# aikiriao/LINNE

Hardware: AMD Instinct MI355X
Metric: frames/sec encode (-m 7) + decode, 44.1 kHz stereo, bit-exact; 1/2/4/8 GPU (higher is better)
Workload: dtype f64; 1 GPU; encode -m 7: 1 x 60 min 44.1 kHz int16 2-channel per GPU = 15504 frames of 10240 samples (tail 9280), MS on, PCM resident in HBM; decode = inverse hot path on the encode output; frames_per_gpu=15504, channels=2, preset=7, tracks_per_gpu=1

## Files before the change

### linne_amd/csrc/lnn_k_finalize.h

```cpp
#ifndef LNN_K_FINALIZE_H_INCLUDED
#define LNN_K_FINALIZE_H_INCLUDED

#define FIN_THREADS 256
#define FIN_TILE (4 * FIN_THREADS)
#define FIN_HALO (LNN_MAXL * LNN_MAXP)

__global__ __launch_bounds__(64) void k_quantize(Plan p)
{
    __shared__ uint32_t s_best;
    const uint32_t cf = blockIdx.x, tid = threadIdx.x;
    const size_t ocf = (size_t)p.frame_map[cf / p.C] * p.C + cf % p.C;
    int32_t *rec = p.prm + ocf * LINNE_AMD_PARAM_WORDS;
    double *st = p.stats + ocf * LINNE_AMD_STAT_WORDS;
    if (tid == 0) {
        double min_loss = (double)FLT_MAX; uint32_t best = 0;
        for (uint32_t r = 0; r < p.R; r++) { const double l = p.jloss[(size_t)cf * p.R + r]; if (l < min_loss) { min_loss = l; best = r; } }
        s_best = best;
        st[LINNE_AMD_ST_TAIL] = p.jtail[(size_t)cf * p.R + best];
        st[LINNE_AMD_ST_BEST] = p.af_best ? (double)p.af_best[cf] : (double)best;
        st[LINNE_AMD_ST_LOSS] = p.af_loss ? p.af_loss[cf] : p.jloss[(size_t)cf * p.R + best];
    }
    uint32_t used = LINNE_AMD_PRM_COEF;
    for (uint32_t l = 0; l < p.L; l++) used += p.P[l];
    for (uint32_t i = LINNE_AMD_PRM_UNITS + tid; i < LINNE_AMD_PARAM_WORDS; i += 64u)
        if ((i >= LINNE_AMD_PRM_UNITS + p.L && i < LINNE_AMD_PRM_RSHIFT) || (i >= LINNE_AMD_PRM_RSHIFT + p.L && i < LINNE_AMD_PRM_COEF) || i >= used) rec[i] = 0;
    __syncthreads();
    const uint32_t job = cf * p.R + s_best;
    __shared__ double s_d[LNN_MAXL][LNN_MAXP];
    for (uint32_t i = tid; i < p.L * LNN_MAXP; i += 64u) { const uint32_t l = i / LNN_MAXP, k = i % LNN_MAXP; if (k < p.P[l]) s_d[l][k] = p.lparams[((size_t)job * LNN_MAXL + l) * LNN_MAXP + k]; }
    __syncthreads();
    if (tid < p.L) {
        const uint32_t l = tid, P = p.P[l];
        const double *d = s_d[l];
        int32_t *cq = rec + LINNE_AMD_PRM_COEF + p.coef_off[l];
        double mx = 0.0;
        for (uint32_t k = 0; k < P; k++) if (mx < fabs(d[k])) mx = fabs(d[k]);
        uint32_t rshift;
        if (mx <= 0.0078125) {
            rshift = 8;
            for (uint32_t k = 0; k < P; k++) cq[k] = 0;
        } else {
            int ndigit; (void)frexp(mx, &ndigit);
            rshift = (uint32_t)(7 - ndigit);
            const double sc = ldexp(1.0, (int)rshift);
            double qerr = 0.0;
            for (int32_t k = (int32_t)P - 1; k >= 0; k--) {
                qerr += d[k] * sc;
                int32_t q = (int32_t)round_away(qerr);
                if (q >= 128) q = 127; else if (q < -128) q = -128;
                qerr -= (double)q;
                cq[k] = q;
            }
        }
        rec[LINNE_AMD_PRM_UNITS + l] = (int32_t)p.lunits[(size_t)job * LNN_MAXL + l];
        rec[LINNE_AMD_PRM_RSHIFT + l] = (int32_t)rshift;
    }
}

#define FIN_FRONT 192u
#define FIN_BUF (FIN_FRONT + ((FIN_HALO + 63u) & ~63u) + FIN_TILE)
__global__ __launch_bounds__(FIN_THREADS, 4) void k_fir_cascade(Plan p)
{
    __shared__ __attribute__((aligned(16))) int32_t s_coef[LNN_MAXL][LNN_MAXP];
    __shared__ __attribute__((aligned(16))) int32_t bufs[2][FIN_BUF];
    __shared__ __attribute__((aligned(16))) int8_t dig[2][4][FIN_BUF];
    const uint32_t cf = blockIdx.x, tid = threadIdx.x;
    const uint32_t lane = tid & 63u, wave = (uint32_t)__builtin_amdgcn_readfirstlane((int)(tid >> 6));
    const DevClass &c = p.cls[p.cls_of_frame[cf / p.C]];
    const uint32_t n = c.n, S = p.S, L = p.L;
    const size_t ocf = (size_t)p.frame_map[cf / p.C] * p.C + cf % p.C;
    const int32_t *rec = p.prm + ocf * LINNE_AMD_PARAM_WORDS;
    int32_t *out = p.resid + ocf * S;
    uint32_t H = 0;
    for (uint32_t l = 0; l < L; l++) H += p.P[l];
    __shared__ uint32_t l_units[LNN_MAXL], l_rs[LNN_MAXL], l_matrix[LNN_MAXL + 1], s_toep_unit[LNN_MAXL];
    __shared__ lnn_v4i s_toep[LNN_MAXL][3][64];
    if (tid <= LNN_MAXL) {
        const uint32_t l = tid;
        if (l < LNN_MAXL) s_toep_unit[l] = 0xFFFFFFFFu;
        uint32_t m = 0;
        if (l < L) {
            const uint32_t units = (uint32_t)rec[LINNE_AMD_PRM_UNITS + l];
            l_units[l] = units; l_rs[l] = (uint32_t)rec[LINNE_AMD_PRM_RSHIFT + l];
            if (l > 0 && units != 0 && p.P[l] <= 128u) { const uint32_t np = p.P[l] / units; m = (np >= 16u && n / units >= np) ? 1u : 0u; }
        }
        l_matrix[l] = m;
    }
    const uint32_t ORG = FIN_FRONT + ((H + 63u) & ~63u);
    const int32_t *src = p.xint + (size_t)cf * S;
    const uint32_t ntile = (S + FIN_TILE - 1u) / FIN_TILE;
    constexpr int NPF = (FIN_HALO + FIN_TILE + FIN_THREADS - 1) / FIN_THREADS;
    int32_t pf[NPF];
    auto fetch = [&](uint32_t s0_) {
#pragma unroll
        for (int m = 0; m < NPF; m++) {
            const uint32_t i = tid + (uint32_t)m * FIN_THREADS;
            const int64_t g = (int64_t)s0_ - H + i;
            pf[m] = (i < H + FIN_TILE && g >= 0 && g < (int64_t)n) ? src[g] : 0;
        }
    };
    if (blockIdx.y < ntile && blockIdx.y * FIN_TILE < n) fetch(blockIdx.y * FIN_TILE);
    for (uint32_t i = tid; i < L * LNN_MAXP; i += FIN_THREADS) { const uint32_t l = i / LNN_MAXP, k = i % LNN_MAXP; if (k < p.P[l]) s_coef[l][k] = rec[LINNE_AMD_PRM_COEF + p.coef_off[l] + k]; }
    for (uint32_t tile = blockIdx.y; tile < ntile; tile += gridDim.y) {
    const uint32_t s0 = tile * FIN_TILE;
    if (s0 >= n) {
        for (uint32_t i = tid; i < FIN_TILE; i += FIN_THREADS) if (s0 + i < S) out[s0 + i] = 0;
        continue;
    }
    __syncthreads();
#pragma unroll
    for (int m = 0; m < NPF; m++) { const uint32_t i = tid + (uint32_t)m * FIN_THREADS; if (i < H + FIN_TILE) bufs[0][ORG - H + i] = pf[m]; }
    { const uint32_t tn = tile + gridDim.y; if (tn < ntile && tn * FIN_TILE < n) fetch(tn * FIN_TILE); }
    __syncthreads();
    uint32_t lead = H;
#pragma unroll 1
    for (uint32_t l = 0; l < L; l++) {
        const uint32_t units = l_units[l], rs = l_rs[l];
        const uint32_t np = p.P[l] / (units ? units : 1u), ns = units ? n / units : 0u;
        const uint32_t half = 1u << ((rs - 1u) & 31u);
        const bool last = (l + 1 == L), digits_out = l_matrix[l + 1] != 0;
        const int32_t *in = bufs[l & 1u];
        int32_t *ob = bufs[(l & 1u) ^ 1u];
        int8_t (*dgo)[FIN_BUF] = dig[(l & 1u) ^ 1u];
        const uint32_t olead = lead - p.P[l];
        const uint32_t count = olead + FIN_TILE;
        const uint32_t nsd = ns ? ns : 1u;
        auto scalar_out = [&](uint32_t idx) -> int32_t {
            const int64_t s64 = (int64_t)s0 - ORG + idx;
            if (s64 < 0 || s64 >= (int64_t)n) return 0;
            const uint32_t s = (uint32_t)s64, unit = s / nsd;
            int32_t v = in[idx];
            if (units && ns >= np && unit < units) {
                const uint32_t loc = s - unit * ns;
                if (loc >= np) {
                    uint32_t pred = half;
                    const int32_t *cc = s_coef[l] + unit * np;
                    const int32_t *xx = in + idx - np;
                    for (uint32_t k = 0; k < np; k++) pred += (uint32_t)cc[k] * (uint32_t)xx[k];
                    v = (int32_t)((uint32_t)v + (uint32_t)((int32_t)pred >> (rs & 31u)));
                }
            }
            return v;
        };
        auto put_digits = [&](uint32_t idx, int32_t v) {
            const uint32_t dg = sp_digits(v);
            dgo[0][idx] = (int8_t)dg; dgo[1][idx] = (int8_t)(dg >> 8); dgo[2][idx] = (int8_t)(dg >> 16); dgo[3][idx] = (int8_t)(dg >> 24);
        };
        if (l_matrix[l] != 0) {
            const uint32_t KS = (np + 15u + 63u) / 64u;
            const int8_t (*dgi)[FIN_BUF] = dig[l & 1u];
            const uint32_t first = (ORG - olead) & ~63u, nchunk = (ORG + FIN_TILE - first) / 64u;
            const uint32_t i = lane & 15u, g4 = lane >> 4, qa = (lane & 15u) >> 2, ba = lane & 3u;
            auto build_band = [&](uint32_t unit, lnn_v4i *frag) {
                const int32_t *cc = s_coef[l] + unit * np;
#pragma unroll
                for (uint32_t st = 0; st < 3u; st++) {
                    uint32_t w[4] = { 0u, 0u, 0u, 0u };
                    if (st < KS) {
#pragma unroll
                        for (uint32_t e = 0; e < 16u; e++) {
                            const int32_t kx = (int32_t)(64u * st + 16u * g4 + e + 16u + np) - (int32_t)(64u * KS + i);
                            const int32_t cv = (kx >= 0 && (uint32_t)kx < np) ? cc[kx] : 0;
                            w[e >> 2] |= ((uint32_t)cv & 0xFFu) << (8u * (e & 3u));
                        }
                    }
                    frag[st][0] = (int)w[0]; frag[st][1] = (int)w[1]; frag[st][2] = (int)w[2]; frag[st][3] = (int)w[3];
                }
            };
            const uint32_t u0 = ((s0 > olead) ? (s0 - olead) / nsd : 0u) < units ? ((s0 > olead) ? (s0 - olead) / nsd : 0u) : units - 1u;
            {
                const uint32_t held = s_toep_unit[l];
                __syncthreads();
                if (held != u0) {
                    if (wave == 0) { lnn_v4i fr[3]; build_band(u0, fr); s_toep[l][0][lane] = fr[0]; s_toep[l][1][lane] = fr[1]; s_toep[l][2][lane] = fr[2]; }
                    if (tid == 0) s_toep_unit[l] = u0;
                }
                __syncthreads();
            }
            lnn_v4i bfrag[3];
            uint32_t have_unit = 0xFFFFFFFFu;
            for (uint32_t ck = wave; ck < nchunk; ck += FIN_THREADS / 64u) {
                const uint32_t bc = first + 64u * ck;
                const int64_t sa = (int64_t)s0 - ORG + bc, sz = sa + 63;
                const uint32_t idx = bc + 16u * g4 + i;
                int32_t o;
                bool mat = sa >= 0 && sz < (int64_t)n;
                uint32_t unit = 0;
                if (mat) { unit = (uint32_t)sa / nsd; mat = unit < units && (uint32_t)sz / nsd == unit; }
                if (mat) {
                    if (unit != have_unit) {
                        if (unit == u0) { bfrag[0] = s_toep[l][0][lane]; bfrag[1] = s_toep[l][1][lane]; bfrag[2] = s_toep[l][2][lane]; }
                        else build_band(unit, bfrag);
                        have_unit = unit;
                    }
                    lnn_v4i acc4 = { 0, 0, 0, 0 };
                    const uint32_t w0 = bc + 16u * qa + 16u - 64u * KS + 16u * g4;
#pragma unroll
                    for (uint32_t st = 0; st < 3u; st++) {
                        if (st < KS) {
                            const lnn_v4i a = *(const lnn_v4i *)&dgi[ba][w0 + 64u * st];
                            acc4 = __builtin_amdgcn_mfma_i32_16x16x64_i8(a, bfrag[st], acc4, 0, 0, 0);
                        }
                    }
                    const uint32_t sum = (uint32_t)acc4[0] + ((uint32_t)acc4[1] << 8) + ((uint32_t)acc4[2] << 16) + ((uint32_t)acc4[3] << 24);
                    const uint32_t s = (uint32_t)((int64_t)s0 - ORG + idx), loc = s - unit * ns;
                    const int32_t v = in[idx];
                    o = (loc >= np) ? (int32_t)((uint32_t)v + (uint32_t)((int32_t)(half + sum) >> (rs & 31u))) : v;
                } else o = scalar_out(idx);
                if (last) { const int64_t s64 = (int64_t)s0 - ORG + idx; if (s64 >= (int64_t)s0 && s64 < (int64_t)S) out[s64] = o; }
                else { ob[idx] = o; if (digits_out) put_digits(idx, o); }
            }
        } else {
        for (uint32_t e0 = 4u * tid; e0 < count; e0 += 4u * FIN_THREADS) {
            const int64_t sb64 = (int64_t)s0 - olead + e0;
            const uint32_t bi = ORG - olead + e0;
            int32_t o[4];
            bool quad = false;
            if (sb64 >= 0 && sb64 + 3 < (int64_t)n && units && ns >= np) {
                const uint32_t sb = (uint32_t)sb64, unit0 = sb / nsd, loc0 = sb - unit0 * nsd;
                quad = (unit0 < units) && (loc0 >= np) && (loc0 + 3 < ns);
                if (quad) {
                    const int32_t *cc = s_coef[l] + unit0 * np;
                    const int32_t *xx = in + bi - np;
                    uint32_t p0 = half, p1 = half, p2 = half, p3 = half;
                    if ((np & 3u) == 0 && ((bi - np) & 3u) == 0) {
                        const int4 *xx4 = (const int4 *)xx, *cc4 = (const int4 *)cc;
                        int4 xa = xx4[0];
                        for (uint32_t k4 = 0; k4 < (np >> 2); k4++) {
                            const int4 xb = xx4[k4 + 1], c4 = cc4[k4];
                            const uint32_t v0 = (uint32_t)xa.x, v1 = (uint32_t)xa.y, v2 = (uint32_t)xa.z, v3 = (uint32_t)xa.w, v4 = (uint32_t)xb.x, v5 = (uint32_t)xb.y, v6 = (uint32_t)xb.z;
                            const uint32_t c0 = (uint32_t)c4.x, c1 = (uint32_t)c4.y, c2 = (uint32_t)c4.z, c3 = (uint32_t)c4.w;
                            p0 += c0 * v0 + c1 * v1 + c2 * v2 + c3 * v3;
                            p1 += c0 * v1 + c1 * v2 + c2 * v3 + c3 * v4;
                            p2 += c0 * v2 + c1 * v3 + c2 * v4 + c3 * v5;
                            p3 += c0 * v3 + c1 * v4 + c2 * v5 + c3 * v6;
                            xa = xb;
                        }
                    } else {
                        uint32_t w0 = (uint32_t)xx[0], w1 = (uint32_t)xx[1], w2 = (uint32_t)xx[2];
                        for (uint32_t k = 0; k < np; k++) {
                            const uint32_t ck = (uint32_t)cc[k], w3 = (uint32_t)xx[k + 3];
                            p0 += ck * w0; p1 += ck * w1; p2 += ck * w2; p3 += ck * w3;
                            w0 = w1; w1 = w2; w2 = w3;
                        }
                    }
                    const int32_t *xv = in + bi;
                    o[0] = (int32_t)((uint32_t)xv[0] + (uint32_t)((int32_t)p0 >> (rs & 31u)));
                    o[1] = (int32_t)((uint32_t)xv[1] + (uint32_t)((int32_t)p1 >> (rs & 31u)));
                    o[2] = (int32_t)((uint32_t)xv[2] + (uint32_t)((int32_t)p2 >> (rs & 31u)));
                    o[3] = (int32_t)((uint32_t)xv[3] + (uint32_t)((int32_t)p3 >> (rs & 31u)));
                }
            }
            if (!quad) { for (uint32_t j = 0; j < 4; j++) o[j] = (e0 + j < count) ? scalar_out(bi + j) : 0; }
            if (last) {
                const uint32_t sb = s0 + e0;
                if (sb + 3 < S && (S & 3u) == 0) { int4 q; q.x = o[0]; q.y = o[1]; q.z = o[2]; q.w = o[3]; *(int4 *)(out + sb) = q; }
                else for (uint32_t j = 0; j < 4; j++) if (sb + j < S) out[sb + j] = o[j];
            } else {
                for (uint32_t j = 0; j < 4; j++) if (e0 + j < count) { ob[bi + j] = o[j]; if (digits_out) put_digits(bi + j, o[j]); }
            }
        }
        }
        lead = olead;
        __syncthreads();
    }
    }
}


#endif
```

Before: 223,700 frames/s.

## Micro-optimize FIR cascade kernel: magic division, uniform loads, mul24, packed digit stores

Precomputes per-layer block sizes and a magic reciprocal so the per-sample divisions become a multiply-high plus correction, and reads per-layer parameters as wave-uniform scalars. When a tile's input fits in 24 bits, the first layer accumulates with __mul24. Digit-plane and sample stores are packed into 32-bit and int4 writes using byte permutes and DPP lane swaps instead of byte-wise scatter. 64-bit index arithmetic is narrowed to 32-bit. These changes add complexity, and the narrow-multiply path depends on a per-tile range check being correct for bit-exactness.

Measured after the change: 223,700 frames/s, median of 2. About the same (+0.0%).

```diff
diff --git a/linne_amd/csrc/lnn_k_finalize.h b/linne_amd/csrc/lnn_k_finalize.h
--- a/linne_amd/csrc/lnn_k_finalize.h
+++ b/linne_amd/csrc/lnn_k_finalize.h
@@ -59,13 +59,51 @@
 
 #define FIN_FRONT 192u
 #define FIN_BUF (FIN_FRONT + ((FIN_HALO + 63u) & ~63u) + FIN_TILE)
+
+__device__ __forceinline__ uint32_t fin_div(uint32_t x, uint32_t d, uint32_t m)
+{
+    const uint32_t q = __umulhi(x, m);
+    return q + ((x - q * d >= d) ? 1u : 0u);
+}
+__device__ __forceinline__ uint32_t fin_uni(uint32_t v) { return (uint32_t)__builtin_amdgcn_readfirstlane((int)v); }
+__device__ __forceinline__ uint32_t fin_perm(uint32_t a, uint32_t b, uint32_t sel) { return __builtin_amdgcn_perm(a, b, sel); }
+
+template <bool NARROW> __device__ __forceinline__ uint32_t fin_mad(uint32_t c, uint32_t x, uint32_t a)
+{
+    return NARROW ? a + (uint32_t)__mul24((int)c, (int)x) : a + c * x;
+}
+template <bool NARROW> __device__ __forceinline__ void fin_quad(const int32_t *cc, const int32_t *xx, uint32_t np, bool vec, uint32_t &p0, uint32_t &p1, uint32_t &p2, uint32_t &p3)
+{
+    if (vec) {
+        const int4 *xx4 = (const int4 *)xx, *cc4 = (const int4 *)cc;
+        int4 xa = xx4[0];
+        for (uint32_t k4 = 0; k4 < (np >> 2); k4++) {
+            const int4 xb = xx4[k4 + 1], c4 = cc4[k4];
+            const uint32_t v0 = (uint32_t)xa.x, v1 = (uint32_t)xa.y, v2 = (uint32_t)xa.z, v3 = (uint32_t)xa.w, v4 = (uint32_t)xb.x, v5 = (uint32_t)xb.y, v6 = (uint32_t)xb.z;
+            const uint32_t c0 = (uint32_t)c4.x, c1 = (uint32_t)c4.y, c2 = (uint32_t)c4.z, c3 = (uint32_t)c4.w;
+            p0 = fin_mad<NARROW>(c3, v3, fin_mad<NARROW>(c2, v2, fin_mad<NARROW>(c1, v1, fin_mad<NARROW>(c0, v0, p0))));
+            p1 = fin_mad<NARROW>(c3, v4, fin_mad<NARROW>(c2, v3, fin_mad<NARROW>(c1, v2, fin_mad<NARROW>(c0, v1, p1))));
+            p2 = fin_mad<NARROW>(c3, v5, fin_mad<NARROW>(c2, v4, fin_mad<NARROW>(c1, v3, fin_mad<NARROW>(c0, v2, p2))));
+            p3 = fin_mad<NARROW>(c3, v6, fin_mad<NARROW>(c2, v5, fin_mad<NARROW>(c1, v4, fin_mad<NARROW>(c0, v3, p3))));
+            xa = xb;
+        }
+    } else {
+        uint32_t w0 = (uint32_t)xx[0], w1 = (uint32_t)xx[1], w2 = (uint32_t)xx[2];
+        for (uint32_t k = 0; k < np; k++) {
+            const uint32_t ck = (uint32_t)cc[k], w3 = (uint32_t)xx[k + 3];
+            p0 = fin_mad<NARROW>(ck, w0, p0); p1 = fin_mad<NARROW>(ck, w1, p1); p2 = fin_mad<NARROW>(ck, w2, p2); p3 = fin_mad<NARROW>(ck, w3, p3);
+            w0 = w1; w1 = w2; w2 = w3;
+        }
+    }
+}
+
 __global__ __launch_bounds__(FIN_THREADS, 4) void k_fir_cascade(Plan p)
 {
     __shared__ __attribute__((aligned(16))) int32_t s_coef[LNN_MAXL][LNN_MAXP];
     __shared__ __attribute__((aligned(16))) int32_t bufs[2][FIN_BUF];
     __shared__ __attribute__((aligned(16))) int8_t dig[2][4][FIN_BUF];
     const uint32_t cf = blockIdx.x, tid = threadIdx.x;
-    const uint32_t lane = tid & 63u, wave = (uint32_t)__builtin_amdgcn_readfirstlane((int)(tid >> 6));
+    const uint32_t lane = tid & 63u, wave = fin_uni(tid >> 6);
     const DevClass &c = p.cls[p.cls_of_frame[cf / p.C]];
     const uint32_t n = c.n, S = p.S, L = p.L;
     const size_t ocf = (size_t)p.frame_map[cf / p.C] * p.C + cf % p.C;
@@ -73,7 +111,7 @@
     int32_t *out = p.resid + ocf * S;
     uint32_t H = 0;
     for (uint32_t l = 0; l < L; l++) H += p.P[l];
-    __shared__ uint32_t l_units[LNN_MAXL], l_rs[LNN_MAXL], l_matrix[LNN_MAXL + 1], s_toep_unit[LNN_MAXL];
+    __shared__ uint32_t l_units[LNN_MAXL], l_rs[LNN_MAXL], l_np[LNN_MAXL], l_ns[LNN_MAXL], l_magic[LNN_MAXL], l_matrix[LNN_MAXL + 1], s_toep_unit[LNN_MAXL], s_wide;
     __shared__ lnn_v4i s_toep[LNN_MAXL][3][64];
     if (tid <= LNN_MAXL) {
         const uint32_t l = tid;
@@ -81,8 +119,10 @@
         uint32_t m = 0;
         if (l < L) {
             const uint32_t units = (uint32_t)rec[LINNE_AMD_PRM_UNITS + l];
+            const uint32_t np = p.P[l] / (units ? units : 1u), ns = units ? n / units : 0u;
             l_units[l] = units; l_rs[l] = (uint32_t)rec[LINNE_AMD_PRM_RSHIFT + l];
-            if (l > 0 && units != 0 && p.P[l] <= 128u) { const uint32_t np = p.P[l] / units; m = (np >= 16u && n / units >= np) ? 1u : 0u; }
+            l_np[l] = np; l_ns[l] = ns; l_magic[l] = 0xFFFFFFFFu / (ns ? ns : 1u);
+            if (l > 0 && units != 0 && p.P[l] <= 128u) m = (np >= 16u && ns >= np) ? 1u : 0u;
         }
         l_matrix[l] = m;
     }
@@ -101,24 +141,30 @@
     };
     if (blockIdx.y < ntile && blockIdx.y * FIN_TILE < n) fetch(blockIdx.y * FIN_TILE);
     for (uint32_t i = tid; i < L * LNN_MAXP; i += FIN_THREADS) { const uint32_t l = i / LNN_MAXP, k = i % LNN_MAXP; if (k < p.P[l]) s_coef[l][k] = rec[LINNE_AMD_PRM_COEF + p.coef_off[l] + k]; }
+    const uint32_t sel_a = (lane & 2u) ? 0x03020706u : 0x05040100u, sel_b = (lane & 1u) ? 0x03070105u : 0x06020400u;
     for (uint32_t tile = blockIdx.y; tile < ntile; tile += gridDim.y) {
     const uint32_t s0 = tile * FIN_TILE;
     if (s0 >= n) {
         for (uint32_t i = tid; i < FIN_TILE; i += FIN_THREADS) if (s0 + i < S) out[s0 + i] = 0;
         continue;
     }
+    if (tid == 0) s_wide = 0u;
     __syncthreads();
-#pragma unroll
-    for (int m = 0; m < NPF; m++) { const uint32_t i = tid + (uint32_t)m * FIN_THREADS; if (i < H + FIN_TILE) bufs[0][ORG - H + i] = pf[m]; }
+    uint32_t mag = 0;
+#pragma unroll
+    for (int m = 0; m < NPF; m++) { const uint32_t i = tid + (uint32_t)m * FIN_THREADS; if (i < H + FIN_TILE) bufs[0][ORG - H + i] = pf[m]; mag |= (uint32_t)(pf[m] ^ (pf[m] >> 31)); }
+    if (mag >> 23) s_wide = 1u;
     { const uint32_t tn = tile + gridDim.y; if (tn < ntile && tn * FIN_TILE < n) fetch(tn * FIN_TILE); }
     __syncthreads();
+    const bool narrow = fin_uni(s_wide) == 0u;
     uint32_t lead = H;
 #pragma unroll 1
     for (uint32_t l = 0; l < L; l++) {
-        const uint32_t units = l_units[l], rs = l_rs[l];
-        const uint32_t np = p.P[l] / (units ? units : 1u), ns = units ? n / units : 0u;
+        const uint32_t units = fin_uni(l_units[l]), rs = fin_uni(l_rs[l]), np = fin_uni(l_np[l]), ns = fin_uni(l_ns[l]), mg = fin_uni(l_magic[l]);
+        const bool matrix = fin_uni(l_matrix[l]) != 0u, digits_out = fin_uni(l_matrix[l + 1]) != 0u;
         const uint32_t half = 1u << ((rs - 1u) & 31u);
-        const bool last = (l + 1 == L), digits_out = l_matrix[l + 1] != 0;
+        const bool last = (l + 1 == L);
+        const bool fast = units != 0u && ns >= np;
         const int32_t *in = bufs[l & 1u];
         int32_t *ob = bufs[(l & 1u) ^ 1u];
         int8_t (*dgo)[FIN_BUF] = dig[(l & 1u) ^ 1u];
@@ -126,11 +172,11 @@
         const uint32_t count = olead + FIN_TILE;
         const uint32_t nsd = ns ? ns : 1u;
         auto scalar_out = [&](uint32_t idx) -> int32_t {
-            const int64_t s64 = (int64_t)s0 - ORG + idx;
-            if (s64 < 0 || s64 >= (int64_t)n) return 0;
-            const uint32_t s = (uint32_t)s64, unit = s / nsd;
+            const int32_t s32 = (int32_t)(s0 + idx) - (int32_t)ORG;
+            if (s32 < 0 || (uint32_t)s32 >= n) return 0;
+            const uint32_t s = (uint32_t)s32, unit = fin_div(s, nsd, mg);
             int32_t v = in[idx];
-            if (units && ns >= np && unit < units) {
+            if (fast && unit < units) {
                 const uint32_t loc = s - unit * ns;
                 if (loc >= np) {
                     uint32_t pred = half;
@@ -146,7 +192,7 @@
             const uint32_t dg = sp_digits(v);
             dgo[0][idx] = (int8_t)dg; dgo[1][idx] = (int8_t)(dg >> 8); dgo[2][idx] = (int8_t)(dg >> 16); dgo[3][idx] = (int8_t)(dg >> 24);
         };
-        if (l_matrix[l] != 0) {
+        if (matrix) {
             const uint32_t KS = (np + 15u + 63u) / 64u;
             const int8_t (*dgi)[FIN_BUF] = dig[l & 1u];
             const uint32_t first = (ORG - olead) & ~63u, nchunk = (ORG + FIN_TILE - first) / 64u;
@@ -167,9 +213,10 @@
                     frag[st][0] = (int)w[0]; frag[st][1] = (int)w[1]; frag[st][2] = (int)w[2]; frag[st][3] = (int)w[3];
                 }
             };
-            const uint32_t u0 = ((s0 > olead) ? (s0 - olead) / nsd : 0u) < units ? ((s0 > olead) ? (s0 - olead) / nsd : 0u) : units - 1u;
+            uint32_t u0 = fin_div((s0 > olead) ? s0 - olead : 0u, nsd, mg);
+            if (u0 >= units) u0 = units - 1u;
             {
-                const uint32_t held = s_toep_unit[l];
+                const uint32_t held = fin_uni(s_toep_unit[l]);
                 __syncthreads();
                 if (held != u0) {
                     if (wave == 0) { lnn_v4i fr[3]; build_band(u0, fr); s_toep[l][0][lane] = fr[0]; s_toep[l][1][lane] = fr[1]; s_toep[l][2][lane] = fr[2]; }
@@ -181,12 +228,12 @@
             uint32_t have_unit = 0xFFFFFFFFu;
             for (uint32_t ck = wave; ck < nchunk; ck += FIN_THREADS / 64u) {
                 const uint32_t bc = first + 64u * ck;
-                const int64_t sa = (int64_t)s0 - ORG + bc, sz = sa + 63;
+                const int32_t sa = (int32_t)(s0 + bc) - (int32_t)ORG;
                 const uint32_t idx = bc + 16u * g4 + i;
                 int32_t o;
-                bool mat = sa >= 0 && sz < (int64_t)n;
+                bool mat = sa >= 0 && (uint32_t)sa + 63u < n;
                 uint32_t unit = 0;
-                if (mat) { unit = (uint32_t)sa / nsd; mat = unit < units && (uint32_t)sz / nsd == unit; }
+                if (mat) { unit = fin_div((uint32_t)sa, nsd, mg); mat = unit < units && (uint32_t)sa + 63u < (unit + 1u) * ns; }
                 if (mat) {
                     if (unit != have_unit) {
                         if (unit == u0) { bfrag[0] = s_toep[l][0][lane]; bfrag[1] = s_toep[l][1][lane]; bfrag[2] = s_toep[l][2][lane]; }
@@ -203,61 +250,72 @@
                         }
                     }
                     const uint32_t sum = (uint32_t)acc4[0] + ((uint32_t)acc4[1] << 8) + ((uint32_t)acc4[2] << 16) + ((uint32_t)acc4[3] << 24);
-                    const uint32_t s = (uint32_t)((int64_t)s0 - ORG + idx), loc = s - unit * ns;
+                    const uint32_t loc = (uint32_t)sa - unit * ns + 16u * g4 + i;
                     const int32_t v = in[idx];
                     o = (loc >= np) ? (int32_t)((uint32_t)v + (uint32_t)((int32_t)(half + sum) >> (rs & 31u))) : v;
                 } else o = scalar_out(idx);
-                if (last) { const int64_t s64 = (int64_t)s0 - ORG + idx; if (s64 >= (int64_t)s0 && s64 < (int64_t)S) out[s64] = o; }
-                else { ob[idx] = o; if (digits_out) put_digits(idx, o); }
+                if (last) { const uint32_t s = s0 + idx - ORG; if (idx >= ORG && s < S) out[s] = o; }
+                else {
+                    ob[idx] = o;
+                    if (digits_out) {
+                        uint32_t t = sp_digits(o);
+                        uint32_t x = (uint32_t)__builtin_amdgcn_update_dpp(0, (int)t, 0x4E, 0xf, 0xf, true);
+                        t = fin_perm(x, t, sel_a);
+                        x = (uint32_t)__builtin_amdgcn_update_dpp(0, (int)t, 0xB1, 0xf, 0xf, true);
+                        t = fin_perm(x, t, sel_b);
+                        *(uint32_t *)&dgo[ba][idx & ~3u] = t;
+                    }
+                }
             }
         } else {
+        const bool al4 = (olead & 3u) == 0u;
         for (uint32_t e0 = 4u * tid; e0 < count; e0 += 4u * FIN_THREADS) {
-            const int64_t sb64 = (int64_t)s0 - olead + e0;
+            const int32_t sb32 = (int32_t)(s0 + e0) - (int32_t)olead;
             const uint32_t bi = ORG - olead + e0;
-            int32_t o[4];
+            int32_t o0 = 0, o1 = 0, o2 = 0, o3 = 0;
             bool quad = false;
-            if (sb64 >= 0 && sb64 + 3 < (int64_t)n && units && ns >= np) {
-                const uint32_t sb = (uint32_t)sb64, unit0 = sb / nsd, loc0 = sb - unit0 * nsd;
+            if (fast && sb32 >= 0 && (uint32_t)sb32 + 3u < n) {
+                const uint32_t sb = (uint32_t)sb32, unit0 = fin_div(sb, nsd, mg), loc0 = sb - unit0 * nsd;
                 quad = (unit0 < units) && (loc0 >= np) && (loc0 + 3 < ns);
                 if (quad) {
                     const int32_t *cc = s_coef[l] + unit0 * np;
                     const int32_t *xx = in + bi - np;
                     uint32_t p0 = half, p1 = half, p2 = half, p3 = half;
-                    if ((np & 3u) == 0 && ((bi - np) & 3u) == 0) {
-                        const int4 *xx4 = (const int4 *)xx, *cc4 = (const int4 *)cc;
-                        int4 xa = xx4[0];
-                        for (uint32_t k4 = 0; k4 < (np >> 2); k4++) {
-                            const int4 xb = xx4[k4 + 1], c4 = cc4[k4];
-                            const uint32_t v0 = (uint32_t)xa.x, v1 = (uint32_t)xa.y, v2 = (uint32_t)xa.z, v3 = (uint32_t)xa.w, v4 = (uint32_t)xb.x, v5 = (uint32_t)xb.y, v6 = (uint32_t)xb.z;
-                            const uint32_t c0 = (uint32_t)c4.x, c1 = (uint32_t)c4.y, c2 = (uint32_t)c4.z, c3 = (uint32_t)c4.w;
-                            p0 += c0 * v0 + c1 * v1 + c2 * v2 + c3 * v3;
-                            p1 += c0 * v1 + c1 * v2 + c2 * v3 + c3 * v4;
-                            p2 += c0 * v2 + c1 * v3 + c2 * v4 + c3 * v5;
-                            p3 += c0 * v3 + c1 * v4 + c2 * v5 + c3 * v6;
-                            xa = xb;
-                        }
-                    } else {
-                        uint32_t w0 = (uint32_t)xx[0], w1 = (uint32_t)xx[1], w2 = (uint32_t)xx[2];
-                        for (uint32_t k = 0; k < np; k++) {
-                            const uint32_t ck = (uint32_t)cc[k], w3 = (uint32_t)xx[k + 3];
-                            p0 += ck * w0; p1 += ck * w1; p2 += ck * w2; p3 += ck * w3;
-                            w0 = w1; w1 = w2; w2 = w3;
-                        }
-                    }
+                    const bool vec = (np & 3u) == 0 && ((bi - np) & 3u) == 0;
+                    if (l == 0 && narrow) fin_quad<true>(cc, xx, np, vec, p0, p1, p2, p3);
+                    else fin_quad<false>(cc, xx, np, vec, p0, p1, p2, p3);
                     const int32_t *xv = in + bi;
-                    o[0] = (int32_t)((uint32_t)xv[0] + (uint32_t)((int32_t)p0 >> (rs & 31u)));
-                    o[1] = (int32_t)((uint32_t)xv[1] + (uint32_t)((int32_t)p1 >> (rs & 31u)));
-                    o[2] = (int32_t)((uint32_t)xv[2] + (uint32_t)((int32_t)p2 >> (rs & 31u)));
-                    o[3] = (int32_t)((uint32_t)xv[3] + (uint32_t)((int32_t)p3 >> (rs & 31u)));
-                }
-            }
-            if (!quad) { for (uint32_t j = 0; j < 4; j++) o[j] = (e0 + j < count) ? scalar_out(bi + j) : 0; }
+                    o0 = (int32_t)((uint32_t)xv[0] + (uint32_t)((int32_t)p0 >> (rs & 31u)));
+                    o1 = (int32_t)((uint32_t)xv[1] + (uint32_t)((int32_t)p1 >> (rs & 31u)));
+                    o2 = (int32_t)((uint32_t)xv[2] + (uint32_t)((int32_t)p2 >> (rs & 31u)));
+                    o3 = (int32_t)((uint32_t)xv[3] + (uint32_t)((int32_t)p3 >> (rs & 31u)));
+                }
+            }
+            if (!quad) {
+                o0 = scalar_out(bi);
+                o1 = (e0 + 1u < count) ? scalar_out(bi + 1u) : 0;
+                o2 = (e0 + 2u < count) ? scalar_out(bi + 2u) : 0;
+                o3 = (e0 + 3u < count) ? scalar_out(bi + 3u) : 0;
+            }
             if (last) {
                 const uint32_t sb = s0 + e0;
-                if (sb + 3 < S && (S & 3u) == 0) { int4 q; q.x = o[0]; q.y = o[1]; q.z = o[2]; q.w = o[3]; *(int4 *)(out + sb) = q; }
-                else for (uint32_t j = 0; j < 4; j++) if (sb + j < S) out[sb + j] = o[j];
+                if (sb + 3 < S && (S & 3u) == 0) { int4 q; q.x = o0; q.y = o1; q.z = o2; q.w = o3; *(int4 *)(out + sb) = q; }
+                else { if (sb < S) out[sb] = o0; if (sb + 1u < S) out[sb + 1u] = o1; if (sb + 2u < S) out[sb + 2u] = o2; if (sb + 3u < S) out[sb + 3u] = o3; }
+            } else if (al4) {
+                int4 q; q.x = o0; q.y = o1; q.z = o2; q.w = o3; *(int4 *)(ob + bi) = q;
+                if (digits_out) {
+                    const uint32_t d0 = sp_digits(o0), d1 = sp_digits(o1), d2 = sp_digits(o2), d3 = sp_digits(o3);
+                    const uint32_t t0 = fin_perm(d1, d0, 0x05010400u), t1 = fin_perm(d3, d2, 0x05010400u);
+                    const uint32_t t2 = fin_perm(d1, d0, 0x07030602u), t3 = fin_perm(d3, d2, 0x07030602u);
+                    *(uint32_t *)&dgo[0][bi] = fin_perm(t1, t0, 0x05040100u);
+                    *(uint32_t *)&dgo[1][bi] = fin_perm(t1, t0, 0x07060302u);
+                    *(uint32_t *)&dgo[2][bi] = fin_perm(t3, t2, 0x05040100u);
+                    *(uint32_t *)&dgo[3][bi] = fin_perm(t3, t2, 0x07060302u);
+                }
             } else {
-                for (uint32_t j = 0; j < 4; j++) if (e0 + j < count) { ob[bi + j] = o[j]; if (digits_out) put_digits(bi + j, o[j]); }
+                const int32_t oo[4] = { o0, o1, o2, o3 };
+#pragma unroll
+                for (uint32_t j = 0; j < 4; j++) if (e0 + j < count) { ob[bi + j] = oo[j]; if (digits_out) put_digits(bi + j, oo[j]); }
             }
         }
         }
```
